# Kmatsuo57/cell-image-analysis

Hardware: AMD Instinct MI355X
Metric: cells/sec screened (CAE fwd + recon-MSE + SVM score), 64x64 (higher is better)
Workload: dtype f32 (results in the fp32 error class; the contractions run as split 16-bit products on the matrix pipe, fp32 accumulate: conv1..conv6 as 2 fp16 terms x 3 products with exact power-of-two scales from each cell's own data, the PCA GEMM as 3 bf16 terms x 6 products, conv7's 32 -> 16 channel contraction; 1 GPU; BASELINE.json configs[2]: screening inference, 1000000 synthetic 64x64 crops on one GPU, resident in HBM, CAE fwd + recon MSE/MAE + RobustScaler + PCA(100) + 2x OCSVM score on device; cells_per_gpu=1000000, global_cells=1000000, chunk_cells=65536, detector_train_cells=5000, weights=random init (Glorot, non-trivial BN), seed 42, parallelism=dp1

## Files before the change

### cell-image-analysis_amd/cellscreen/_lib.py

```python
from __future__ import annotations

import ctypes as C
import os
from typing import Optional

import numpy as np

CS_MAX_CONV = 16
CS_MEM_HOST, CS_MEM_DEVICE = 0, 1
_PKG = os.path.dirname(os.path.dirname(os.path.abspath(__file__)))
LIB_PATH = os.path.join(_PKG, "libcellscreen.so")


class CellScreenError(RuntimeError):
    def __init__(self, status: int, message: str):
        super().__init__(f"libcellscreen status {status}: {message}")
        self.status = status


class CSAugAffine(C.Structure):
    _fields_ = [("m", C.c_double * 4), ("off", C.c_double * 2), ("identity", C.c_int32), ("flip_h", C.c_int32),
                ("flip_v", C.c_int32), ("reserved", C.c_int32)]


# ... 24 lines not shown
                ("conservative", CSOcsvmParams), ("moderate", CSOcsvmParams)]


ALLGATHER_FN = C.CFUNCTYPE(C.c_int, C.c_void_p, C.c_int64)
ALLGATHER_STREAM_FN = C.CFUNCTYPE(C.c_int, C.c_void_p, C.c_int64, C.c_void_p)


class CSTrainCfg(C.Structure):
    _fields_ = [("beta1", C.c_float), ("beta2", C.c_float), ("adam_eps", C.c_float),
                ("bn_momentum", C.c_float), ("bn_eps", C.c_float)]


PRECISION_SPLIT16, PRECISION_FP32_EXACT = 0, 1
PRECISIONS = {"split16": PRECISION_SPLIT16, "fp32_exact": PRECISION_FP32_EXACT, "exact": PRECISION_FP32_EXACT,
              PRECISION_SPLIT16: PRECISION_SPLIT16, PRECISION_FP32_EXACT: PRECISION_FP32_EXACT}
DEBUG_NO_FUSE12, DEBUG_NO_FUSE45, DEBUG_NO_FUSE67, DEBUG_NO_SMALL_SPLIT = 1, 2, 4, 8


class CSModelOptions(C.Structure):
    _fields_ = [("struct_size", C.c_uint32), ("precision", C.c_int32), ("debug_flags", C.c_uint32), ("reserved", C.c_uint32 * 5)]


def model_options(precision="split16", debug_flags: int = 0) -> "CSModelOptions":
    if precision not in PRECISIONS:
        raise ValueError(f"precision must be 'split16' or 'fp32_exact', got {precision!r}")
    o = CSModelOptions()
    o.struct_size = C.sizeof(CSModelOptions)
    o.precision = PRECISIONS[precision]
    o.debug_flags = int(debug_flags)
    return o

# ... 335 lines not shown
```

### cell-image-analysis_amd/csrc/api.hip

```cpp
#include "api_internal.hpp"
#include "tensor_archive.hpp"

using namespace cs;

static thread_local std::string g_err;

namespace cs {
int fail(int code, const char* fmt, ...)
{
    char buf[1024];
    va_list ap;
    va_start(ap, fmt);
    vsnprintf(buf, sizeof buf, fmt, ap);
    va_end(ap);
    g_err = buf;
    return code;
}
const char* last_error_cstr() { return g_err.c_str(); }
}

static const char* kKernelNames[K_COUNT] = {"conv1_relu_bn_pool", "conv2_relu_bn_pool", "conv3_relu_bn_pool",
                                            "conv4_relu_bn",      "conv5_up_relu_bn",   "conv6_up_relu_bn",
                                            "conv7_up_sigmoid_err", "scaler_pca",       "ocsvm_decision",
                                            "finalize",           "synth_crops",        "conv6_conv7_fused_err",
                                            "conv1_conv2_fused"};

struct ConvSet {
    DevBuf winocs[3];
    DevBuf c12w1;
    DevBuf c3h2, c4h2, c5h2, c6h2;
    float c3h2_inv = 1.0f, c4h2_inv = 1.0f, c5h2_inv = 1.0f, c6h2_inv = 1.0f;
    DevBuf c12w1h2;
    float c12w1h2_inv = 1.0f;
    DevBuf c12h2;
    float c12h2_inv = 1.0f, p1a = 0.0f, p1b = 0.0f;
    DevBuf c12;
    DevBuf winoup[6];
    DevBuf wfrag[6];
    DevBuf ep[6];
    int n = 0;
};

struct GenSet {
    DevBuf w[CS_MAX_CONV], ep[CS_MAX_CONV], wf[CS_MAX_CONV], wx3[CS_MAX_CONV];
    bool folded[CS_MAX_CONV] = {false}, x3[CS_MAX_CONV] = {false};
    DevBuf wh2[CS_MAX_CONV];
// ... 15 lines not shown

constexpr int64_t kPackedResultCells = 65536;

struct cs_model {
    int device = 0;
    hipStream_t stream = nullptr;
    hipStream_t copy_stream = nullptr;
    hipEvent_t ev_in[2] = {nullptr, nullptr}, ev_used[2] = {nullptr, nullptr};
    Arch arch;
    ConvSet ae, enc;
    GenSet gae, genc;
    bool shared_encoder = true;
    int precision = CS_PRECISION_SPLIT16;
    unsigned debug_flags = 0;
    bool split16 = true;
    bool fuse12 = true, fuse45 = true, fuse67 = true, small_split = true;
    int errparts = 4;
    DevBuf w7eff, b7;
    bool has_det = false;
    int F = 0, fpad = 0, C = 0, cpad = 0;
    DevBuf center, scale, comps, comps_x3, mean_proj;
    struct Svm { DevBuf svT, svn, coef; int nsv = 0, nsv_pad = 0; double gamma = 0, rho = 0; } svm[2];
    int64_t chunk = 0;
    int64_t ws_cells = 0;
    DevBuf xin, xin2, act[CS_MAX_CONV], featE, pca, errpart, dec[2], o_mse, o_mae, o_sc[2], o_pr[2], recon;
    DevBuf det_ws;
    DevBuf o_pack;
    void* h_pack = nullptr;
    size_t h_pack_bytes = 0;
    bool prof = false;
    std::vector<ProfEvent> pending;
// ... 152 lines not shown
        }
        if (l == 4) {
            std::vector<float> weff(pack_generic_folded(cin, cout, nullptr, nullptr));
            pack_generic_folded(cin, cout, w->kernel[l], weff.data());
            std::vector<uint16_t> h2(pack_conv5_f16x2(nullptr, nullptr, nullptr));
            pack_conv5_f16x2(weff.data(), h2.data(), &set.c5h2_inv);
            rc = upload(set.c5h2, h2.data(), h2.size() * sizeof(uint16_t));
            if (rc) return rc;
        }
        if (l == 5) {
            std::vector<float> weff(pack_generic_folded(cin, cout, nullptr, nullptr));
            pack_generic_folded(cin, cout, w->kernel[l], weff.data());
            std::vector<uint16_t> h2(pack_conv6_f16x2(nullptr, nullptr, nullptr));
            pack_conv6_f16x2(weff.data(), h2.data(), &set.c6h2_inv);
            rc = upload(set.c6h2, h2.data(), h2.size() * sizeof(uint16_t));
            if (rc) return rc;
        }
        if (l == 0) {
            tmp.resize(pack_conv12_conv1_fragments(nullptr, nullptr, nullptr));
            pack_conv12_conv1_fragments(w->kernel[l], ep.data() + cout, tmp.data());
            rc = upload(set.c12w1, tmp.data(), tmp.size() * sizeof(float));
            if (rc) return rc;
            pack_conv12_p1_bound(w->kernel[l], ep.data(), &set.p1a, &set.p1b);
            std::vector<unsigned int> wh(pack_conv12_conv1_h2(nullptr, nullptr, nullptr, nullptr));
            pack_conv12_conv1_h2(w->kernel[l], ep.data() + cout, wh.data(), &set.c12w1h2_inv);
            rc = upload(set.c12w1h2, wh.data(), wh.size() * sizeof(unsigned int));
            if (rc) return rc;
        }
        if (l == 1) {
            tmp.resize(pack_conv12_fragments(nullptr, nullptr, nullptr));
// ... 260 lines not shown
        if (l == 1 || l == 2) {
            LAUNCH(K_CONV1 + l, nc,
                   launch_conv_wino_cs(l, in, set.winocs[l].as<float>(), set.ep[l].as<float>(), m->act[l].as<float>(), nc, m->stream));
            continue;
        }
        if (l == 3 && h2) {
            LAUNCH(K_CONV4, nc,
                   launch_conv4_h2(in, set.c4h2.as<uint16_t>(), set.c4h2_inv, set.ep[l].as<float>(), m->act[l].as<float>(), nc, m->stream));
            continue;
        }
        LAUNCH(K_CONV1 + l, nc,
               launch_conv_mfma(l, in, set.wfrag[l].as<float>(), set.ep[l].as<float>(), m->act[l].as<float>(), nc, m->stream, false));
    }
    if (fused && h2) {
        LAUNCH(K_CONV67_FUSED, nc,
               launch_conv67_h2(m->act[4].as<float>(), set.c6h2.as<uint16_t>(), set.c6h2_inv, set.ep[5].as<float>(), x, m->w7eff.as<float>(),
                                m->b7.as<float>(), m->errpart.as<float>(), nc, m->stream));
        m->errparts = conv67_fused_nparts();
    } else if (fused) {
        LAUNCH(K_CONV67_FUSED, nc,
               launch_conv67_fused(m->act[4].as<float>(), set.winoup[5].as<float>(), set.ep[5].as<float>(), x, m->w7eff.as<float>(),
                                   m->b7.as<float>(), m->errpart.as<float>(), nc, m->stream));
        m->errparts = conv67_fused_nparts();
    } else if (last >= 6) {
        LAUNCH(K_CONV7_ERR, nc,
               launch_conv7_err(m->act[5].as<float>(), x, m->w7eff.as<float>(), m->b7.as<float>(), m->errpart.as<float>(), recon, nc, m->stream));
        m->errparts = 4;
    }
    return CS_OK;
}

struct DrainGuard {
// ... 81 lines not shown
int cs_device_count(void)
{
    int n = 0;
    if (hipGetDeviceCount(&n) != hipSuccess) return 0;
    return n;
}

static int resolve_options(const cs_model_options* o, int* precision, unsigned* flags)
{
    *precision = CS_PRECISION_SPLIT16;
    *flags = 0;
    if (o) {
        if (o->struct_size < 12 || o->struct_size > 4096) return fail(CS_ERR_INVALID, "cs_model_options.struct_size = %u (set it to sizeof(cs_model_options))", o->struct_size);
        if (o->precision != CS_PRECISION_SPLIT16 && o->precision != CS_PRECISION_FP32_EXACT)
            return fail(CS_ERR_INVALID, "cs_model_options.precision = %d (CS_PRECISION_SPLIT16 or CS_PRECISION_FP32_EXACT)", o->precision);
        const unsigned known = CS_DEBUG_NO_FUSE12 | CS_DEBUG_NO_FUSE45 | CS_DEBUG_NO_FUSE67 | CS_DEBUG_NO_SMALL_SPLIT;
        if (o->debug_flags & ~known) return fail(CS_ERR_INVALID, "cs_model_options.debug_flags = 0x%x has unknown bits", o->debug_flags);
        if (o->struct_size >= sizeof(cs_model_options))
            for (unsigned r : o->reserved) if (r) return fail(CS_ERR_INVALID, "cs_model_options.reserved must be 0");
        *precision = o->precision;
        *flags = o->debug_flags;
    }
    if (const char* e = getenv("CS_DEBUG_PRECISION")) {
        if (!strcmp(e, "exact")) *precision = CS_PRECISION_FP32_EXACT;
        else if (!strcmp(e, "split16")) *precision = CS_PRECISION_SPLIT16;
        else return fail(CS_ERR_INVALID, "CS_DEBUG_PRECISION=%s (exact or split16)", e);
    }
    if (const char* e = getenv("CS_DEBUG_FLAGS")) *flags |= (unsigned)strtoul(e, nullptr, 0) & 0xfu;
    return CS_OK;
}

int cs_model_from_arrays(const cs_cae_weights* autoencoder, const cs_cae_weights* encoder,
                         const cs_detector_params* det, int device_id, const cs_model_options* options, cs_model** out)
{
    if (!out) return fail(CS_ERR_INVALID, "out is NULL");
    *out = nullptr;
    int precision;
    unsigned dflags;
    {
        int rco = resolve_options(options, &precision, &dflags);
        if (rco) return rco;
    }
    Arch arch;
// ... 2 lines not shown
    if (arch.ref && (rc = check_arch(autoencoder, kNConv, "autoencoder"))) return rc;
    if (encoder && (rc = check_encoder(encoder, arch))) return rc;
    if ((rc = require_gfx950(device_id))) return rc;

    cs_model* m = new (std::nothrow) cs_model();
    if (!m) return fail(CS_ERR_NOMEM, "host allocation failed");
    m->device = device_id;
    m->arch = arch;
    m->precision = precision;
    m->debug_flags = dflags;
    m->split16 = precision == CS_PRECISION_SPLIT16;
    m->fuse12 = !(dflags & CS_DEBUG_NO_FUSE12);
    m->fuse45 = !(dflags & CS_DEBUG_NO_FUSE45);
    m->fuse67 = !(dflags & CS_DEBUG_NO_FUSE67);
    m->small_split = !(dflags & CS_DEBUG_NO_SMALL_SPLIT);
#define FAIL_IF(x) do { int r__ = (x); if (r__) { delete m; return r__; } } while (0)
    {
        hipError_t e = hipStreamCreateWithFlags(&m->stream, hipStreamNonBlocking);
        if (e == hipSuccess) e = hipStreamCreateWithFlags(&m->copy_stream, hipStreamNonBlocking);
        for (int i = 0; i < 2 && e == hipSuccess; ++i) {
            e = hipEventCreateWithFlags(&m->ev_in[i], hipEventDisableTiming);
            if (e == hipSuccess) e = hipEventCreateWithFlags(&m->ev_used[i], hipEventDisableTiming);
        }
        if (e != hipSuccess) { delete m; return fail(CS_ERR_HIP, "stream/event creation: %s", hipGetErrorString(e)); }
    }
    if (arch.ref) {
        FAIL_IF(pack_set(m->ae, autoencoder, 6));
        float weff[16 * 32];
        conv7_effective_weights(autoencoder->kernel[6], weff);
        FAIL_IF(upload(m->w7eff, weff, sizeof weff));
// ... 549 lines not shown

int cs_profile_bf16_mfma_per_cell(cs_model* m, int k, double* mfma)
{
    if (!m || !mfma || k < 0 || k >= K_COUNT) return fail(CS_ERR_INVALID, "bad kernel id");
    double v = 0.0;
    if (!m->split16) { *mfma = 0.0; return CS_OK; }
    if (k == K_SCALER_PCA && m->has_det) {
        *mfma = (double)(m->cpad / 16) * (m->fpad / 32) * 6.0 / 16.0;
        return CS_OK;
    }
    if (m->arch.ref) {
        if (k == K_CONV4) v = 4 * 2 * 9 * 3;
        if (k == K_CONV3) v = 16.0 * 4 * 2 * 2 * 3;
        if (k == K_CONV12_FUSED) v = 66 * 8 * 2 + 36 * 4 * 4 * 3;
        if (k == K_CONV5) v = 4 * 4 * 4 * 4 * 3 + (m->fuse45 ? 4 * 2 * 9 * 3 : 0);
        if (k == K_CONV67_FUSED) v = 4.0 * 16 * 2 * 4 * 2 * 3;
    } else if (k <= K_CONV6) {
        const int l = k - K_CONV1;
        if (l < m->arch.n_conv && m->gae.x3[l]) {
            const int cout_pad = (m->arch.ch[l] + 15) / 16 * 16;
            const double taps = l > m->arch.n_enc ? 4.0 : 9.0;
            const bool last = l == m->arch.n_conv - 1;
            v = (double)m->arch.gh[l] * m->arch.gw[l] / 16.0 * (cout_pad / 16) * taps * (m->arch.cin(l) / 32.0) * ((m->gae.h2_inv[l] != 0.0f && !last) ? 3.0 : 6.0);
        }
    }
    *mfma = v;
    return CS_OK;
}

}
```

### cell-image-analysis_amd/csrc/common.hpp

```cpp
#pragma once
#include <hip/hip_runtime.h>
#include <stdint.h>
#include <stdio.h>

#include "../../include/cellscreen.h"

namespace cs {

typedef float f32x4 __attribute__((ext_vector_type(4)));

struct LayerGeom {
    int H, W, cin, cout;
    bool pool;
    bool ups;
    bool last;
};

enum KernelId {
    K_CONV1 = 0, K_CONV2, K_CONV3, K_CONV4, K_CONV5, K_CONV6, K_CONV7_ERR,
    K_SCALER_PCA, K_SVM, K_FINALIZE, K_SYNTH, K_CONV67_FUSED, K_CONV12_FUSED, K_COUNT
};

hipError_t launch_conv_mfma(int layer, const float* in, const float* wfrag, const float* ep,
                            float* out, int64_t n_cells, hipStream_t stream, bool folded = false);
// ... 14 lines not shown
size_t pack_conv12_conv1_fragments(const float* hwio, const float* bn_scale, float* dst);
hipError_t launch_conv4_h2(const float* in, const uint16_t* wfrag, float inv_sw, const float* ep, float* out, int64_t n_cells, hipStream_t stream);
size_t pack_conv4_f16x2(const float* hwio, uint16_t* dst, float* inv_sw);
hipError_t launch_conv5_h2(const float* in, const uint16_t* wfrag, float inv_sw, const float* ep, float* out, int64_t n_cells, hipStream_t stream);
hipError_t launch_conv45_h2(const float* in, const uint16_t* w4, float inv_sw4, const float* ep4, const uint16_t* w5, float inv_sw5,
                            const float* ep5, float* out, int64_t n_cells, hipStream_t stream);
size_t pack_conv5_f16x2(const float* weff, uint16_t* dst, float* inv_sw);
hipError_t launch_conv_wino_up(int layer, const float* in, const float* ufrag, const float* ep, float* out, int64_t n_cells,
                               hipStream_t stream);
size_t pack_wino_up_fragments(int layer, const float* hwio, float* dst);
size_t pack_conv_fragments(int cin, int cout, const float* hwio, float* dst);

hipError_t launch_conv67_fused(const float* a5, const float* ufrag, const float* ep, const float* x, const float* weff_dev,
                               const float* b7_dev, float* errpart, int64_t n_cells, hipStream_t stream);
int conv67_fused_nparts();
hipError_t launch_conv67_h2(const float* a5, const uint16_t* wplanes, float inv_sw, const float* ep, const float* x, const float* weff_dev,
                            const float* b7_dev, float* errpart, int64_t n_cells, hipStream_t stream);
size_t pack_conv6_f16x2(const float* weff, uint16_t* dst, float* inv_sw);

hipError_t launch_conv7_err(const float* a6, const float* x, const float* weff_dev, const float* b7_dev,
                            float* errpart, float* recon, int64_t n_cells, hipStream_t stream);
hipError_t launch_conv7_err_train(const float* a6, const float* x, const float* weff_dev, const float* b7_dev, float* errpart,
                                  float* recon, float* dz, float* dzsum_part, int64_t n_cells, hipStream_t stream);
void conv7_effective_weights(const float* w7_hwio, float* weff);

constexpr int TRAIN_MAX_PARTS = 256;
constexpr int BN_MAX_PARTS = 1024;
struct ReduceDesc { long dst; long len; const float* src; int nparts; long stride; };
hipError_t launch_conv_train_fwd(int layer, const float* in, const float* wfrag, const float* bias,
                                 float* relu_out, int64_t n_cells, hipStream_t stream, float* stats_part = nullptr,
                                 int* stats_parts = nullptr);
hipError_t launch_conv_dgrad(int layer, const float* dz, const float* wfrag_t, float* dx, int64_t n_cells,
                             hipStream_t stream);
// ... 84 lines not shown
```

### cell-image-analysis_amd/csrc/conv_wino_up.hip

```cpp
#include "kernel_setup.hpp"
#include "split16.hpp"

#include <type_traits>

#include <cmath>
#include <cstdlib>
#include <cstring>

namespace cs {

namespace {

template <int HS_, int WS_, int CIN_, int COUT_>
struct WUCfg {
    static constexpr int HS = HS_, WS = WS_, CIN = CIN_, COUT = COUT_;
    static constexpr int HO = 2 * HS, WO = 2 * WS;
    static constexpr int TW = WS / 2;
    static constexpr int SR = 2 * (16 / TW);
    static constexpr int R = SR + 2, WP = WS + 2;
    static constexpr int PS = CIN + 4;
    static constexpr int STRIP = R * WP * PS * 4;
    static constexpr int LDS = 2 * STRIP;
    static constexpr int NGRP = HS / SR;
    static constexpr int NQ = CIN / 16, KS = CIN / 4;
// ... 393 lines not shown

struct F67H {
    static constexpr int PLB = 2 * 64;
    static constexpr int PXB = 2 * PLB + 32;
    static constexpr int ROWB = 18 * PXB;
    static constexpr int STRIP = 6 * ROWB;
    static constexpr int TW = F67T::TW;
    static constexpr int T_BYTES = F67T::T_BYTES;
    static constexpr int PA = 40;
    static constexpr int A6_BYTES = 8 * 32 * PA * 4;
    static constexpr int WP = 40;
    static constexpr int W_BYTES = 16 * WP * 4;
    static constexpr int OFF_MAX = STRIP + A6_BYTES + T_BYTES + W_BYTES;
    static constexpr int LDS = OFF_MAX + 16;
    static_assert(LDS <= 160 * 1024 && STRIP % 16 == 0, "LDS budget");
};

__device__ __forceinline__ void h2_store(char* strip, int j, int rsub, int loffb, const f32x4& v, float S)
{
    const int r = rsub + WUL6::RPP * j;
    f16x4 hi, lo;
    f16x2_split4(v, S, hi, lo);
    char* d = strip + r * F67H::ROWB + loffb;
    *(f16x4*)d = hi;
    *(f16x4*)(d + F67H::PLB) = lo;
}

__device__ __forceinline__ f32x4 h2_prep(int y0, int j, int rsub, f32x4 v, unsigned int& mx)
{
    const int sy = y0 - 1 + rsub + WUL6::RPP * j;
    if (sy < 0 || sy >= WUL6::HS) v = f32x4{0.0f, 0.0f, 0.0f, 0.0f};
    f16x2_absmax4(v, mx);
    return v;
}

template <bool DIAG>
__global__ __launch_bounds__(WUL6::THREADS, 2) void conv67_h2_kernel(
    const float* __restrict__ in , const f16x8* __restrict__ wfrag, const float* __restrict__ ep ,
    const float* __restrict__ x , const float* __restrict__ weff ,
    const float* __restrict__ b7p, float* __restrict__ errpart , long n_cells, float inv_sw,
    unsigned long long* __restrict__ diag)
{
    using C = WUL6;
    static_assert(C::NLD == 3 && C::RPP == 2 && C::R == 6 && C::EPR == 256, "row-wise staging constants");
    unsigned long long dg[5] = {0, 0, 0, 0, 0}, dt = 0;
    extern __shared__ __attribute__((aligned(16))) char smem[];
    float* a6s = (float*)(smem + F67H::STRIP);
    float* tb = (float*)(smem + F67H::STRIP + F67H::A6_BYTES);
    float* wl = (float*)(smem + F67H::STRIP + F67H::A6_BYTES + F67H::T_BYTES);
    unsigned int* mxw = (unsigned int*)(smem + F67H::OFF_MAX);
    const int tid = threadIdx.x, lane = tid & 63;
    const int wave = __builtin_amdgcn_readfirstlane(tid >> 6);
    const int ph = wave >> 1, wsl = wave & 1;
    const int pa = ph >> 1, pb = ph & 1;
    const int li = lane & 15, kq = lane >> 4;

    f16x8 B[4][2][2];
#pragma unroll
    for (int t = 0; t < 4; ++t)
#pragma unroll
        for (int k = 0; k < 2; ++k)
#pragma unroll
            for (int p = 0; p < 2; ++p) B[t][k][p] = wfrag[(((wave * 4 + t) * 2 + k) * 2 + p) * 64 + lane];
    const int co = wsl * 16 + li;
    const int cosw = co ^ ((kq & 1) << 4);
    const float bias = ep[co], bns = ep[C::COUT + co], bnt = ep[2 * C::COUT + co];
    const float b7 = b7p[0];

    const long first = blockIdx.x;
    if (first >= n_cells) return;
    const int se = tid & (C::EPR - 1), rsub = tid / C::EPR;
    const int spx = se / C::C4, sc4 = se & (C::C4 - 1);
    const int goff = spx * C::CIN + sc4 * 4;
    const int loffb = (spx + 1) * F67H::PXB + sc4 * 8;
    auto cell_ptr = [&](long cell) { return in + (size_t)cell * C::HS * C::WS * C::CIN; };
    for (int i = tid; i < F67H::LDS / 16; i += C::THREADS) ((f32x4*)smem)[i] = f32x4{0.0f, 0.0f, 0.0f, 0.0f};
    __syncthreads();
    wl[(tid >> 5) * F67H::WP + (tid & 31)] = weff[tid];
    float unscale;
    {
        f32x4 stg[C::NLD];
        unsigned int mx = 0;
#pragma unroll
        for (int j = 0; j < C::NLD; ++j) stg[j] = h2_prep(0, j, rsub, wu_load<C>(cell_ptr(first), 0, j, rsub, goff), mx);
        mx = f16x2_rowmax(mx);
        if (li == 0) atomicMax(&mxw[0], mx);
        __syncthreads();
        float S, invS;
        f16x2_scale(mxw[0], S, invS);
        unscale = invS * inv_sw;
#pragma unroll
        for (int j = 0; j < C::NLD; ++j) h2_store(smem, j, rsub, loffb, stg[j], S);
    }
    __syncthreads();
    if (tid == 0) mxw[0] = 0;
    const char* abase = smem + (pa * 18 + li + pb) * F67H::PXB + kq * 16;

    int strip_no = 0;
    for (long cell = first; cell < n_cells; cell += gridDim.x) {
        const float* xc = x + (size_t)cell * 64 * 64;
        float s2 = 0.0f, s1 = 0.0f;
#pragma unroll 1
        for (int grp = 0; grp < C::NGRP; ++grp) {
            const long ncell = grp < C::NGRP - 1 ? cell : cell + gridDim.x;
            const int ngrp = grp < C::NGRP - 1 ? grp + 1 : 0;
            const bool has_next = ncell < n_cells;
            ++strip_no;
            unsigned int* const mword = mxw + (strip_no & 1);

            if constexpr (DIAG) dt = cycle_stamp();
            f32x4 stg[C::NLD];
            if (has_next) {
#pragma unroll
                for (int j = 0; j < C::NLD; ++j) stg[j] = wu_load<C>(cell_ptr(ncell), ngrp * C::SR, j, rsub, goff);
            }
            float xv[2];
#pragma unroll
            for (int h = 0; h < 2; ++h) {
                const int k = wave + 8 * h, o = 2 * (8 * grp + (k >> 1)) - 1 + (k & 1);
                xv[h] = xc[(o < 0 ? 0 : o) * 64 + lane];
            }
            float xtail = 0.0f;
            if (grp == C::NGRP - 1 && wave == 0) xtail = xc[63 * 64 + lane];

            if constexpr (DIAG) { const unsigned long long t = cycle_stamp(); dg[0] += t - dt; dt = t; }
            f32x4 ah[4], al[4];
#pragma unroll
            for (int t = 0; t < 4; ++t) ah[t] = al[t] = f32x4{0.0f, 0.0f, 0.0f, 0.0f};
            auto rd = [&](int f, f16x8 (&a)[2]) {
                const int sr = f >> 2, rx = (f >> 1) & 1, k = f & 1;
                const char* p = abase + sr * F67H::ROWB + rx * F67H::PXB + k * 64;
                a[0] = *(const f16x8*)p;
                a[1] = *(const f16x8*)(p + F67H::PLB);
            };
            auto mac3 = [&](const f16x8 (&a)[2], const f16x8 (&b)[2], f32x4& dh, f32x4& dl) {
                dl = __builtin_amdgcn_mfma_f32_16x16x32_f16(a[0], b[1], dl, 0, 0, 0);
                dh = __builtin_amdgcn_mfma_f32_16x16x32_f16(a[0], b[0], dh, 0, 0, 0);
                dl = __builtin_amdgcn_mfma_f32_16x16x32_f16(a[1], b[0], dl, 0, 0, 0);
            };
            {
// ... 12 lines not shown
                    if (sr > 0 && sr < 4) __builtin_amdgcn_sched_group_barrier(0x008, 6, 0);
                    else __builtin_amdgcn_sched_group_barrier(0x008, 3, 0);
                }
            }
            if constexpr (DIAG) {
                asm volatile("" ::"v"(ah[0][0]), "v"(al[3][3]));
                const unsigned long long t = cycle_stamp(); dg[1] += t - dt; dt = t;
            }
#pragma unroll
            for (int t = 0; t < 4; ++t)
#pragma unroll
                for (int r = 0; r < 4; ++r) {
                    const float v = fmaxf(fmaf(ah[t][r] + al[t][r], unscale, bias), 0.0f);
                    a6s[((2 * t + pa) * 32 + 2 * (4 * kq + r) + pb) * F67H::PA + cosw] = fmaf(v, bns, bnt);
                }
            if (has_next) {
                unsigned int mx = 0;
#pragma unroll
                for (int j = 0; j < C::NLD; ++j) stg[j] = h2_prep(ngrp * C::SR, j, rsub, stg[j], mx);
                mx = f16x2_rowmax(mx);
                if (li == 0) atomicMax(mword, mx);
            }
            __syncthreads();
            if constexpr (DIAG) { const unsigned long long t = cycle_stamp(); dg[2] += t - dt; dt = t; }
            {
                const int wrow = 4 * ((li >> 3) | (((li >> 2) & 1) << 1)) + (li & 3);
                float wc[8];
                *(f32x4*)&wc[0] = *(const f32x4*)(wl + wrow * F67H::WP + 4 * kq);
                *(f32x4*)&wc[4] = *(const f32x4*)(wl + wrow * F67H::WP + 4 * kq + 16);
                const int pix = 4 * (li & 3) + (li >> 2), sw = ((li >> 1) & 1) << 4;
                const float* ap = a6s + (wave * 32 + pix) * F67H::PA + 4 * kq;
                const f32x4 a00 = *(const f32x4*)(ap + sw), a01 = *(const f32x4*)(ap + (sw ^ 16));
                const f32x4 a10 = *(const f32x4*)(ap + 16 * F67H::PA + sw), a11 = *(const f32x4*)(ap + 16 * F67H::PA + (sw ^ 16));
                f32x4 t0 = f32x4{0.0f, 0.0f, 0.0f, 0.0f}, t1 = t0;
#pragma unroll
                for (int s = 0; s < 4; ++s) {
                    t0 = __builtin_amdgcn_mfma_f32_16x16x4f32(wc[s], a00[s], t0, 0, 0, 0);
                    t1 = __builtin_amdgcn_mfma_f32_16x16x4f32(wc[s], a10[s], t1, 0, 0, 0);
                }
#pragma unroll
                for (int s = 0; s < 4; ++s) {
                    t0 = __builtin_amdgcn_mfma_f32_16x16x4f32(wc[4 + s], a01[s], t0, 0, 0, 0);
                    t1 = __builtin_amdgcn_mfma_f32_16x16x4f32(wc[4 + s], a11[s], t1, 0, 0, 0);
                }
                const int rblk = kq == 0 ? 0 : (kq == 1 ? 3 : (kq == 2 ? 1 : 2));
                float* tw = tb + ((((8 * grp + wave) & (F67::TSLOTS - 1)) * 16) + 4 * rblk) * F67H::TW + pix + 1 - (kq >> 1);
#pragma unroll
                for (int r = 0; r < 4; ++r) { tw[r * F67H::TW] = t0[r]; tw[r * F67H::TW + 16] = t1[r]; }
            }
            if (has_next) {
                float S, invS;
                f16x2_scale(*mword, S, invS);
                unscale = invS * inv_sw;
#pragma unroll
                for (int j = 0; j < C::NLD; ++j) h2_store(smem, j, rsub, loffb, stg[j], S);
            }
            __syncthreads();
            if (tid == 0) *mword = 0;
            if constexpr (DIAG) { const unsigned long long t = cycle_stamp(); dg[3] += t - dt; dt = t; }
            const int px = lane & 1, xh = lane >> 1;
#pragma unroll
            for (int h = 0; h < 2; ++h) {
                const int k = wave + 8 * h;
                const int y = 8 * grp + (k >> 1), e = k & 1;
                if (2 * y - 1 + e < 0) continue;
                const int nb = (e ? px : 3 - px) * 4;
                const float* ra = tb + ((((y - 1) & (F67::TSLOTS - 1)) * 16) + nb) * F67H::TW + xh;
                const float* rb = tb + (((y & (F67::TSLOTS - 1)) * 16) + nb) * F67H::TW + xh;
// ... 8 lines not shown
            }
            if (grp == C::NGRP - 1 && wave == 0) {
                const int nb = (3 - px) * 4;
                const float* ra = tb + (((31 & (F67::TSLOTS - 1)) * 16) + nb) * F67H::TW + xh;
                const float v = (ra[0] + ra[F67H::TW + 1]) + b7;
                const float rr = f67_sigmoid(v);
                const float d = xtail - rr;
                s2 = fmaf(d, d, s2);
                s1 += fabsf(d);
            }
            if constexpr (DIAG) {
                asm volatile("" ::"v"(s2), "v"(s1));
                const unsigned long long t = cycle_stamp(); dg[4] += t - dt; dt = t;
            }
        }
#pragma unroll
        for (int off = 32; off > 0; off >>= 1) {
            s2 += __shfl_down(s2, off, 64);
            s1 += __shfl_down(s1, off, 64);
        }
        if (lane == 0) {
            errpart[((size_t)cell * F67::NPARTS + wave) * 2 + 0] = s2;
            errpart[((size_t)cell * F67::NPARTS + wave) * 2 + 1] = s1;
        }
    }
    if constexpr (DIAG) {
        if (lane == 0) {
#pragma unroll
            for (int k = 0; k < 5; ++k) diag[((size_t)blockIdx.x * 8 + wave) * 5 + k] = dg[k];
        }
    }
}

template <class C>
// ... 80 lines not shown
    if (inv_sw) *inv_sw = 1.0f / S;
    for (int w = 0; w < 8; ++w)
        for (int t = 0; t < 4; ++t)
            for (int k = 0; k < 2; ++k)
                for (int l = 0; l < 64; ++l)
                    for (int j = 0; j < 8; ++j) {
                        const int ph = w >> 1, half = w & 1, li = l & 15, kq = l >> 4;
                        const float v = weff[((size_t)(ph * 4 + t) * 64 + 32 * k + 8 * kq + j) * 32 + 16 * half + li];
                        uint16_t pl[2];
                        f16x2_split(v, S, pl[0], pl[1]);
                        for (int p = 0; p < 2; ++p) dst[((((((size_t)w * 4 + t) * 2 + k) * 2 + p) * 64) + l) * 8 + j] = pl[p];
                    }
    return n;
}

hipError_t launch_conv67_h2(const float* a5, const uint16_t* wplanes, float inv_sw, const float* ep, const float* x, const float* weff_dev,
                            const float* b7_dev, float* errpart, int64_t n_cells, hipStream_t stream)
{
    static const bool diag = getenv("CS_WINO_DIAG") != nullptr;
    KernelSetup ks;
    const hipError_t e = !diag ? kernel_setup<conv67_h2_kernel<false>>(WUL6::THREADS, F67H::LDS, ks)
                               : kernel_setup<conv67_h2_kernel<true>>(WUL6::THREADS, F67H::LDS, ks, &g_wu_stamps[0]);
    if (e != hipSuccess) return e;
    if (n_cells <= 0) return hipSuccess;
    const unsigned grid = (unsigned)(n_cells < ks.cus ? n_cells : ks.cus);
    if (diag)
        hipLaunchKernelGGL(conv67_h2_kernel<true>, dim3(grid), dim3(WUL6::THREADS), F67H::LDS, stream, a5, (const f16x8*)wplanes, ep, x,
                           weff_dev, b7_dev, errpart, (long)n_cells, inv_sw, g_wu_stamps[0].begin(ks, grid));
    else
        hipLaunchKernelGGL(conv67_h2_kernel<false>, dim3(grid), dim3(WUL6::THREADS), F67H::LDS, stream, a5, (const f16x8*)wplanes, ep, x,
                           weff_dev, b7_dev, errpart, (long)n_cells, inv_sw, (unsigned long long*)nullptr);
    return hipGetLastError();
}

size_t pack_wino_up_fragments(int layer, const float* hwio, float* dst)
{
    return layer == 5 ? pack_frags<WUL6>(hwio, dst) : pack_frags<WUL5>(hwio, dst);
}

hipError_t launch_conv_wino_up(int layer, const float* in, const float* ufrag, const float* ep, float* out, int64_t n_cells,
                               hipStream_t stream)
{
    if (layer == 5) return launch<WUL6>(layer, in, ufrag, ep, out, n_cells, stream);
    if (layer == 4) return launch<WUL5>(layer, in, ufrag, ep, out, n_cells, stream);
    return hipErrorInvalidValue;
}

}

extern "C" int cs_debug_wino_up_diag(int layer, double out5[5])
{
    if (layer < 3 || layer > 5) return -1;
    return cs::stamp_table_average(cs::g_wu_stamps[layer - 3], 5, out5);
}
```

### include/cellscreen.h

```cpp
#ifndef CELLSCREEN_H
#define CELLSCREEN_H

#include <stdint.h>

#ifdef __cplusplus
extern "C" {
#endif

#define CS_ABI_VERSION 2
#define CS_MAX_CONV 16

typedef enum cs_status {
    CS_OK = 0,
    CS_ERR_INVALID = -1,
    CS_ERR_IO = -2,
    CS_ERR_FORMAT = -3,
    CS_ERR_NO_DEVICE = -4,
    CS_ERR_HIP = -5,
    CS_ERR_UNSUPPORTED = -6,
    CS_ERR_NOMEM = -7,
    CS_ERR_NO_DETECTOR = -8
} cs_status;

typedef enum cs_mem_kind { CS_MEM_HOST = 0, CS_MEM_DEVICE = 1 } cs_mem_kind;
// ... 26 lines not shown
    int32_t n_components;
    const float *scaler_center;
    const double *scaler_scale;
    const float *pca_components;
    const float *pca_mean_proj;
    cs_ocsvm_params conservative;
    cs_ocsvm_params moderate;
} cs_detector_params;

typedef enum cs_precision { CS_PRECISION_SPLIT16 = 0, CS_PRECISION_FP32_EXACT = 1 } cs_precision;

#define CS_DEBUG_NO_FUSE12      0x1u
#define CS_DEBUG_NO_FUSE45      0x2u
#define CS_DEBUG_NO_FUSE67      0x4u
#define CS_DEBUG_NO_SMALL_SPLIT 0x8u

typedef struct cs_model_options {
    uint32_t struct_size;
    int32_t precision;
    uint32_t debug_flags;
    uint32_t reserved[5];
} cs_model_options;

typedef struct cs_model_info {
    int32_t height, width;
    int32_t n_conv, n_enc;
    int32_t feature_dim;
    int32_t n_components;
    int32_t n_sv_conservative, n_sv_moderate;
    int32_t shared_encoder;
// ... 456 lines not shown
```

Before: 5.563 million cells/s.

## Compute fused conv6 upsample as nine direct taps with cross-wave halo exchange

Adds a new default path for the fused conv6+conv7 kernel. It packs the conv6 weights per tap (9 taps) instead of the folded 4-phase sub-pixel form. Each wave computes tap products on its input row, combines horizontal neighbours with DPP lane shifts, and swaps vertical halo rows with other waves through a new LDS area. The aim is to cut the MFMA count per cell relative to the folded-phase formulation. The change also adds a swizzled LDS channel layout, epilogue params staged in LDS and a ds_swizzle reduction, at the cost of more LDS, an extra barrier and more complex scale handling across groups.

New measurement: 5.506 million cells/s. -1.0%, worse.

```diff
diff --git a/cell-image-analysis_amd/cellscreen/_lib.py b/cell-image-analysis_amd/cellscreen/_lib.py
--- a/cell-image-analysis_amd/cellscreen/_lib.py
+++ b/cell-image-analysis_amd/cellscreen/_lib.py
@@ -62,7 +62,7 @@
 PRECISION_SPLIT16, PRECISION_FP32_EXACT = 0, 1
 PRECISIONS = {"split16": PRECISION_SPLIT16, "fp32_exact": PRECISION_FP32_EXACT, "exact": PRECISION_FP32_EXACT,
               PRECISION_SPLIT16: PRECISION_SPLIT16, PRECISION_FP32_EXACT: PRECISION_FP32_EXACT}
-DEBUG_NO_FUSE12, DEBUG_NO_FUSE45, DEBUG_NO_FUSE67, DEBUG_NO_SMALL_SPLIT = 1, 2, 4, 8
+DEBUG_NO_FUSE12, DEBUG_NO_FUSE45, DEBUG_NO_FUSE67, DEBUG_NO_SMALL_SPLIT, DEBUG_NO_TAPS67 = 1, 2, 4, 8, 0x20
 
 
 class CSModelOptions(C.Structure):
diff --git a/cell-image-analysis_amd/csrc/api.hip b/cell-image-analysis_amd/csrc/api.hip
--- a/cell-image-analysis_amd/csrc/api.hip
+++ b/cell-image-analysis_amd/csrc/api.hip
@@ -30,6 +30,8 @@
     DevBuf c12w1;
     DevBuf c3h2, c4h2, c5h2, c6h2;
     float c3h2_inv = 1.0f, c4h2_inv = 1.0f, c5h2_inv = 1.0f, c6h2_inv = 1.0f;
+    DevBuf c6t;
+    float c6t_inv = 1.0f;
     DevBuf c12w1h2;
     float c12w1h2_inv = 1.0f;
     DevBuf c12h2;
@@ -75,7 +77,7 @@
     int precision = CS_PRECISION_SPLIT16;
     unsigned debug_flags = 0;
     bool split16 = true;
-    bool fuse12 = true, fuse45 = true, fuse67 = true, small_split = true;
+    bool fuse12 = true, fuse45 = true, fuse67 = true, small_split = true, taps67 = true;
     int errparts = 4;
     DevBuf w7eff, b7;
     bool has_det = false;
@@ -258,6 +260,10 @@
             std::vector<uint16_t> h2(pack_conv6_f16x2(nullptr, nullptr, nullptr));
             pack_conv6_f16x2(weff.data(), h2.data(), &set.c6h2_inv);
             rc = upload(set.c6h2, h2.data(), h2.size() * sizeof(uint16_t));
+            if (rc) return rc;
+            std::vector<uint16_t> t9(pack_conv6_taps_f16x2(nullptr, nullptr, nullptr));
+            pack_conv6_taps_f16x2(w->kernel[l], t9.data(), &set.c6t_inv);
+            rc = upload(set.c6t, t9.data(), t9.size() * sizeof(uint16_t));
             if (rc) return rc;
         }
         if (l == 0) {
@@ -548,8 +554,8 @@
     }
     if (fused && h2) {
         LAUNCH(K_CONV67_FUSED, nc,
-               launch_conv67_h2(m->act[4].as<float>(), set.c6h2.as<uint16_t>(), set.c6h2_inv, set.ep[5].as<float>(), x, m->w7eff.as<float>(),
-                                m->b7.as<float>(), m->errpart.as<float>(), nc, m->stream));
+               launch_conv67_h2(m->act[4].as<float>(), (m->taps67 ? set.c6t : set.c6h2).as<uint16_t>(), m->taps67 ? set.c6t_inv : set.c6h2_inv,
+                                m->taps67, set.ep[5].as<float>(), x, m->w7eff.as<float>(), m->b7.as<float>(), m->errpart.as<float>(), nc, m->stream));
         m->errparts = conv67_fused_nparts();
     } else if (fused) {
         LAUNCH(K_CONV67_FUSED, nc,
@@ -661,7 +667,7 @@
         if (o->struct_size < 12 || o->struct_size > 4096) return fail(CS_ERR_INVALID, "cs_model_options.struct_size = %u (set it to sizeof(cs_model_options))", o->struct_size);
         if (o->precision != CS_PRECISION_SPLIT16 && o->precision != CS_PRECISION_FP32_EXACT)
             return fail(CS_ERR_INVALID, "cs_model_options.precision = %d (CS_PRECISION_SPLIT16 or CS_PRECISION_FP32_EXACT)", o->precision);
-        const unsigned known = CS_DEBUG_NO_FUSE12 | CS_DEBUG_NO_FUSE45 | CS_DEBUG_NO_FUSE67 | CS_DEBUG_NO_SMALL_SPLIT;
+        const unsigned known = CS_DEBUG_NO_FUSE12 | CS_DEBUG_NO_FUSE45 | CS_DEBUG_NO_FUSE67 | CS_DEBUG_NO_SMALL_SPLIT | CS_DEBUG_NO_TAPS67;
         if (o->debug_flags & ~known) return fail(CS_ERR_INVALID, "cs_model_options.debug_flags = 0x%x has unknown bits", o->debug_flags);
         if (o->struct_size >= sizeof(cs_model_options))
             for (unsigned r : o->reserved) if (r) return fail(CS_ERR_INVALID, "cs_model_options.reserved must be 0");
@@ -673,7 +679,7 @@
         else if (!strcmp(e, "split16")) *precision = CS_PRECISION_SPLIT16;
         else return fail(CS_ERR_INVALID, "CS_DEBUG_PRECISION=%s (exact or split16)", e);
     }
-    if (const char* e = getenv("CS_DEBUG_FLAGS")) *flags |= (unsigned)strtoul(e, nullptr, 0) & 0xfu;
+    if (const char* e = getenv("CS_DEBUG_FLAGS")) *flags |= (unsigned)strtoul(e, nullptr, 0) & 0x2fu;
     return CS_OK;
 }
 
@@ -706,6 +712,7 @@
     m->fuse45 = !(dflags & CS_DEBUG_NO_FUSE45);
     m->fuse67 = !(dflags & CS_DEBUG_NO_FUSE67);
     m->small_split = !(dflags & CS_DEBUG_NO_SMALL_SPLIT);
+    m->taps67 = !(dflags & CS_DEBUG_NO_TAPS67);
 #define FAIL_IF(x) do { int r__ = (x); if (r__) { delete m; return r__; } } while (0)
     {
         hipError_t e = hipStreamCreateWithFlags(&m->stream, hipStreamNonBlocking);
@@ -1285,7 +1292,7 @@
         if (k == K_CONV3) v = 16.0 * 4 * 2 * 2 * 3;
         if (k == K_CONV12_FUSED) v = 66 * 8 * 2 + 36 * 4 * 4 * 3;
         if (k == K_CONV5) v = 4 * 4 * 4 * 4 * 3 + (m->fuse45 ? 4 * 2 * 9 * 3 : 0);
-        if (k == K_CONV67_FUSED) v = 4.0 * 16 * 2 * 4 * 2 * 3;
+        if (k == K_CONV67_FUSED) v = conv67_h2_mfma_per_cell(m->taps67);
     } else if (k <= K_CONV6) {
         const int l = k - K_CONV1;
         if (l < m->arch.n_conv && m->gae.x3[l]) {
diff --git a/cell-image-analysis_amd/csrc/common.hpp b/cell-image-analysis_amd/csrc/common.hpp
--- a/cell-image-analysis_amd/csrc/common.hpp
+++ b/cell-image-analysis_amd/csrc/common.hpp
@@ -52,9 +52,11 @@
 hipError_t launch_conv67_fused(const float* a5, const float* ufrag, const float* ep, const float* x, const float* weff_dev,
                                const float* b7_dev, float* errpart, int64_t n_cells, hipStream_t stream);
 int conv67_fused_nparts();
-hipError_t launch_conv67_h2(const float* a5, const uint16_t* wplanes, float inv_sw, const float* ep, const float* x, const float* weff_dev,
-                            const float* b7_dev, float* errpart, int64_t n_cells, hipStream_t stream);
+hipError_t launch_conv67_h2(const float* a5, const uint16_t* wplanes, float inv_sw, bool taps, const float* ep, const float* x,
+                            const float* weff_dev, const float* b7_dev, float* errpart, int64_t n_cells, hipStream_t stream);
 size_t pack_conv6_f16x2(const float* weff, uint16_t* dst, float* inv_sw);
+size_t pack_conv6_taps_f16x2(const float* hwio, uint16_t* dst, float* inv_sw);
+int conv67_h2_mfma_per_cell(bool taps);
 
 hipError_t launch_conv7_err(const float* a6, const float* x, const float* weff_dev, const float* b7_dev,
                             float* errpart, float* recon, int64_t n_cells, hipStream_t stream);
diff --git a/cell-image-analysis_amd/csrc/conv_wino_up.hip b/cell-image-analysis_amd/csrc/conv_wino_up.hip
--- a/cell-image-analysis_amd/csrc/conv_wino_up.hip
+++ b/cell-image-analysis_amd/csrc/conv_wino_up.hip
@@ -431,7 +431,37 @@
     static constexpr int OFF_MAX = STRIP + A6_BYTES + T_BYTES + W_BYTES;
     static constexpr int LDS = OFF_MAX + 16;
     static_assert(LDS <= 160 * 1024 && STRIP % 16 == 0, "LDS budget");
+    __device__ static __forceinline__ int chan(int col, int c0) { return c0 ^ (((col >> 3) & 1) << 4); }
 };
+
+struct F67N {
+    static constexpr int PA = 32;
+    static constexpr int A6_BYTES = 8 * 32 * PA * 4;
+    static constexpr int XCH_SLOT = 64 * 16;
+    static constexpr int XCH_BYTES = 34 * XCH_SLOT;
+    static constexpr int OFF_XCH = F67H::STRIP + A6_BYTES + F67H::T_BYTES + F67H::W_BYTES;
+    static constexpr int OFF_EP = OFF_XCH + XCH_BYTES;
+    static constexpr int OFF_MAX = OFF_EP + 3 * 32 * 4;
+    static constexpr int LDS = OFF_MAX + 16;
+    static constexpr int MFMA_PER_CELL = 4 * (8 * 54 + 2 * 18);
+    static_assert(LDS <= 160 * 1024, "LDS budget");
+    __device__ static __forceinline__ int chan(int col, int c0)
+    {
+        return c0 ^ ((((col >> 2) & 1) << 2) | (((col >> 1) & 1) << 3) | (((col >> 3) & 1) << 4));
+    }
+};
+
+template <bool SHR>
+__device__ __forceinline__ float row_neighbour(float v)
+{
+    return __builtin_bit_cast(float, __builtin_amdgcn_update_dpp(0, __builtin_bit_cast(int, v), SHR ? 0x111 : 0x101, 0xf, 0xf, true));
+}
+
+template <int M>
+__device__ __forceinline__ float lane_xor(float v)
+{
+    return __builtin_bit_cast(float, __builtin_amdgcn_ds_swizzle(__builtin_bit_cast(int, v), (M << 10) | 0x1f));
+}
 
 __device__ __forceinline__ void h2_store(char* strip, int j, int rsub, int loffb, const f32x4& v, float S)
 {
@@ -451,7 +481,7 @@
     return v;
 }
 
-template <bool DIAG>
+template <bool DIAG, bool TAPS>
 __global__ __launch_bounds__(WUL6::THREADS, 2) void conv67_h2_kernel(
     const float* __restrict__ in , const f16x8* __restrict__ wfrag, const float* __restrict__ ep ,
     const float* __restrict__ x , const float* __restrict__ weff ,
@@ -459,28 +489,30 @@
     unsigned long long* __restrict__ diag)
 {
     using C = WUL6;
+    using L = std::conditional_t<TAPS, F67N, F67H>;
     static_assert(C::NLD == 3 && C::RPP == 2 && C::R == 6 && C::EPR == 256, "row-wise staging constants");
     unsigned long long dg[5] = {0, 0, 0, 0, 0}, dt = 0;
     extern __shared__ __attribute__((aligned(16))) char smem[];
     float* a6s = (float*)(smem + F67H::STRIP);
-    float* tb = (float*)(smem + F67H::STRIP + F67H::A6_BYTES);
-    float* wl = (float*)(smem + F67H::STRIP + F67H::A6_BYTES + F67H::T_BYTES);
-    unsigned int* mxw = (unsigned int*)(smem + F67H::OFF_MAX);
+    float* tb = (float*)(smem + F67H::STRIP + L::A6_BYTES);
+    float* wl = (float*)(smem + F67H::STRIP + L::A6_BYTES + F67H::T_BYTES);
+    unsigned int* mxw = (unsigned int*)(smem + L::OFF_MAX);
     const int tid = threadIdx.x, lane = tid & 63;
     const int wave = __builtin_amdgcn_readfirstlane(tid >> 6);
     const int ph = wave >> 1, wsl = wave & 1;
     const int pa = ph >> 1, pb = ph & 1;
     const int li = lane & 15, kq = lane >> 4;
 
-    f16x8 B[4][2][2];
-#pragma unroll
-    for (int t = 0; t < 4; ++t)
+    constexpr int NT = TAPS ? 9 : 4;
+    f16x8 B[NT][2][2];
+#pragma unroll
+    for (int t = 0; t < NT; ++t)
 #pragma unroll
         for (int k = 0; k < 2; ++k)
 #pragma unroll
-            for (int p = 0; p < 2; ++p) B[t][k][p] = wfrag[(((wave * 4 + t) * 2 + k) * 2 + p) * 64 + lane];
+            for (int p = 0; p < 2; ++p) B[t][k][p] = wfrag[((((TAPS ? wsl : wave) * NT + t) * 2 + k) * 2 + p) * 64 + lane];
     const int co = wsl * 16 + li;
-    const int cosw = co ^ ((kq & 1) << 4);
+    const int cosw = F67H::chan(8 * kq, co);
     const float bias = ep[co], bns = ep[C::COUT + co], bnt = ep[2 * C::COUT + co];
     const float b7 = b7p[0];
 
@@ -491,9 +523,12 @@
     const int goff = spx * C::CIN + sc4 * 4;
     const int loffb = (spx + 1) * F67H::PXB + sc4 * 8;
     auto cell_ptr = [&](long cell) { return in + (size_t)cell * C::HS * C::WS * C::CIN; };
-    for (int i = tid; i < F67H::LDS / 16; i += C::THREADS) ((f32x4*)smem)[i] = f32x4{0.0f, 0.0f, 0.0f, 0.0f};
+    for (int i = tid; i < L::LDS / 16; i += C::THREADS) ((f32x4*)smem)[i] = f32x4{0.0f, 0.0f, 0.0f, 0.0f};
     __syncthreads();
     wl[(tid >> 5) * F67H::WP + (tid & 31)] = weff[tid];
+    if constexpr (TAPS) {
+        if (tid < 3 * C::COUT) ((float*)(smem + F67N::OFF_EP))[tid] = ep[tid];
+    }
     float unscale;
     {
         f32x4 stg[C::NLD];
@@ -505,13 +540,15 @@
         __syncthreads();
         float S, invS;
         f16x2_scale(mxw[0], S, invS);
-        unscale = invS * inv_sw;
+        unscale = TAPS ? __builtin_bit_cast(float, __builtin_amdgcn_readfirstlane(__builtin_bit_cast(int, invS * inv_sw))) : invS * inv_sw;
 #pragma unroll
         for (int j = 0; j < C::NLD; ++j) h2_store(smem, j, rsub, loffb, stg[j], S);
     }
     __syncthreads();
     if (tid == 0) mxw[0] = 0;
-    const char* abase = smem + (pa * 18 + li + pb) * F67H::PXB + kq * 16;
+    const char* abase = TAPS ? smem + ((ph + 1) * 18 + li + 1) * F67H::PXB + kq * 16 : smem + (pa * 18 + li + pb) * F67H::PXB + kq * 16;
+    f32x4* const xch = (f32x4*)(smem + F67N::OFF_XCH) + lane;
+    float* const a6w = a6s + (2 * ph * 32 + 2 * li) * F67N::PA + F67N::chan(2 * li, 16 * wsl + 4 * kq);
 
     int strip_no = 0;
     for (long cell = first; cell < n_cells; cell += gridDim.x) {
@@ -531,16 +568,112 @@
 #pragma unroll
                 for (int j = 0; j < C::NLD; ++j) stg[j] = wu_load<C>(cell_ptr(ncell), ngrp * C::SR, j, rsub, goff);
             }
-            float xv[2];
-#pragma unroll
-            for (int h = 0; h < 2; ++h) {
-                const int k = wave + 8 * h, o = 2 * (8 * grp + (k >> 1)) - 1 + (k & 1);
-                xv[h] = xc[(o < 0 ? 0 : o) * 64 + lane];
-            }
-            float xtail = 0.0f;
-            if (grp == C::NGRP - 1 && wave == 0) xtail = xc[63 * 64 + lane];
+            float xv[2], xtail = 0.0f;
+            auto load_x = [&]() {
+#pragma unroll
+                for (int h = 0; h < 2; ++h) {
+                    const int k = wave + 8 * h, o = 2 * (8 * grp + (k >> 1)) - 1 + (k & 1);
+                    xv[h] = xc[(unsigned)((o < 0 ? 0 : o) * 64 + lane)];
+                }
+                if constexpr (TAPS) {
+                    if (wave == 0) xtail = xc[(unsigned)((16 * grp + 15) * 64 + lane)];
+                } else if (grp == C::NGRP - 1 && wave == 0) xtail = xc[63 * 64 + lane];
+            };
+            if constexpr (!TAPS) load_x();
 
             if constexpr (DIAG) { const unsigned long long t = cycle_stamp(); dg[0] += t - dt; dt = t; }
+            if constexpr (TAPS) {
+            const int t = ph;
+            f16x8 xa[2][2];
+#pragma unroll
+            for (int k = 0; k < 2; ++k)
+#pragma unroll
+                for (int p = 0; p < 2; ++p) xa[k][p] = *(const f16x8*)(abase + k * 64 + p * F67H::PLB);
+            f32x4 z[9];
+#pragma unroll
+            for (int j = 0; j < 9; ++j) z[j] = f32x4{0.0f, 0.0f, 0.0f, 0.0f};
+#pragma unroll
+            for (int s = 0; s < 3; ++s)
+#pragma unroll
+                for (int k = 0; k < 2; ++k)
+#pragma unroll
+                    for (int j = 0; j < 9; ++j)
+                        z[j] = __builtin_amdgcn_mfma_f32_16x16x32_f16(B[j][k][s == 0], xa[k][s == 1], z[j], 0, 0, 0);
+            f32x4 c[3][2];
+#pragma unroll
+            for (int i = 0; i < 3; ++i)
+#pragma unroll
+                for (int r = 0; r < 4; ++r) {
+                    c[i][0][r] = row_neighbour<true>(z[3 * i][r]) + (z[3 * i + 1][r] + z[3 * i + 2][r]);
+                    c[i][1][r] = (z[3 * i][r] + z[3 * i + 1][r]) + row_neighbour<false>(z[3 * i + 2][r]);
+                }
+            {
+                const int s0 = t < 3 ? (t * 2 + wsl) * 2 : 12 + ((grp & 1) * 2 + wsl) * 2;
+                const float cs = t < 3 ? 1.0f : unscale;
+                xch[64 * s0] = c[0][0] * cs;
+                xch[64 * (s0 + 1)] = c[0][1] * cs;
+                if (t > 0) {
+                    xch[64 * (20 + ((t - 1) * 2 + wsl) * 2)] = c[2][0];
+                    xch[64 * (20 + ((t - 1) * 2 + wsl) * 2 + 1)] = c[2][1];
+                }
+            }
+            f32x4 up[2], dn[2];
+            if (t == 3) {
+#pragma unroll
+                for (int k = 0; k < 2; ++k)
+#pragma unroll
+                    for (int p = 0; p < 2; ++p) xa[k][p] = *(const f16x8*)(abase + F67H::ROWB + k * 64 + p * F67H::PLB);
+                f32x4 zh[3];
+#pragma unroll
+                for (int j = 0; j < 3; ++j) zh[j] = f32x4{0.0f, 0.0f, 0.0f, 0.0f};
+#pragma unroll
+                for (int s = 0; s < 3; ++s)
+#pragma unroll
+                    for (int k = 0; k < 2; ++k)
+#pragma unroll
+                        for (int j = 0; j < 3; ++j)
+                            zh[j] = __builtin_amdgcn_mfma_f32_16x16x32_f16(B[6 + j][k][s == 0], xa[k][s == 1], zh[j], 0, 0, 0);
+#pragma unroll
+                for (int r = 0; r < 4; ++r) {
+                    dn[0][r] = row_neighbour<true>(zh[0][r]) + (zh[1][r] + zh[2][r]);
+                    dn[1][r] = (zh[0][r] + zh[1][r]) + row_neighbour<false>(zh[2][r]);
+                }
+            }
+            if constexpr (DIAG) {
+                asm volatile("" ::"v"(c[1][0][0]), "v"(c[1][1][3]));
+                const unsigned long long ts = cycle_stamp(); dg[1] += ts - dt; dt = ts;
+            }
+            __syncthreads();
+            {
+                const int su = t > 0 ? ((t - 1) * 2 + wsl) * 2 : (grp > 0 ? 12 + (((grp - 1) & 1) * 2 + wsl) * 2 : 32);
+                up[0] = xch[64 * su];
+                up[1] = xch[64 * (su + 1)];
+                if (t == 0 && grp > 0) {
+                    const float rs = __builtin_bit_cast(float, 0x7f000000u - __builtin_bit_cast(unsigned int, unscale));
+                    up[0] *= rs;
+                    up[1] *= rs;
+                }
+            }
+            if (t < 3) {
+                dn[0] = xch[64 * (20 + (t * 2 + wsl) * 2)];
+                dn[1] = xch[64 * (20 + (t * 2 + wsl) * 2 + 1)];
+            }
+            const f32x4* const ep4 = (const f32x4*)(smem + F67N::OFF_EP) + 4 * wsl + kq;
+            const f32x4 bias4 = ep4[0], bns4 = ep4[8], bnt4 = ep4[16];
+#pragma unroll
+            for (int a = 0; a < 2; ++a)
+#pragma unroll
+                for (int b = 0; b < 2; ++b) {
+                    f32x4 o;
+#pragma unroll
+                    for (int r = 0; r < 4; ++r) {
+                        const float s = a == 0 ? up[b][r] + (c[1][b][r] + c[2][b][r]) : (c[0][b][r] + c[1][b][r]) + dn[b][r];
+                        o[r] = fmaf(fmaxf(fmaf(s, unscale, bias4[r]), 0.0f), bns4[r], bnt4[r]);
+                    }
+                    *(f32x4*)(a6w + (a * 32 + b) * F67N::PA) = o;
+                }
+            load_x();
+            } else {
             f32x4 ah[4], al[4];
 #pragma unroll
             for (int t = 0; t < 4; ++t) ah[t] = al[t] = f32x4{0.0f, 0.0f, 0.0f, 0.0f};
@@ -583,6 +716,7 @@
                     const float v = fmaxf(fmaf(ah[t][r] + al[t][r], unscale, bias), 0.0f);
                     a6s[((2 * t + pa) * 32 + 2 * (4 * kq + r) + pb) * F67H::PA + cosw] = fmaf(v, bns, bnt);
                 }
+            }
             if (has_next) {
                 unsigned int mx = 0;
 #pragma unroll
@@ -597,10 +731,10 @@
                 float wc[8];
                 *(f32x4*)&wc[0] = *(const f32x4*)(wl + wrow * F67H::WP + 4 * kq);
                 *(f32x4*)&wc[4] = *(const f32x4*)(wl + wrow * F67H::WP + 4 * kq + 16);
-                const int pix = 4 * (li & 3) + (li >> 2), sw = ((li >> 1) & 1) << 4;
-                const float* ap = a6s + (wave * 32 + pix) * F67H::PA + 4 * kq;
+                const int pix = 4 * (li & 3) + (li >> 2), sw = L::chan(pix, 4 * kq);
+                const float* ap = a6s + (wave * 32 + pix) * L::PA;
                 const f32x4 a00 = *(const f32x4*)(ap + sw), a01 = *(const f32x4*)(ap + (sw ^ 16));
-                const f32x4 a10 = *(const f32x4*)(ap + 16 * F67H::PA + sw), a11 = *(const f32x4*)(ap + 16 * F67H::PA + (sw ^ 16));
+                const f32x4 a10 = *(const f32x4*)(ap + 16 * L::PA + sw), a11 = *(const f32x4*)(ap + 16 * L::PA + (sw ^ 16));
                 f32x4 t0 = f32x4{0.0f, 0.0f, 0.0f, 0.0f}, t1 = t0;
 #pragma unroll
                 for (int s = 0; s < 4; ++s) {
@@ -620,7 +754,7 @@
             if (has_next) {
                 float S, invS;
                 f16x2_scale(*mword, S, invS);
-                unscale = invS * inv_sw;
+                unscale = TAPS ? __builtin_bit_cast(float, __builtin_amdgcn_readfirstlane(__builtin_bit_cast(int, invS * inv_sw))) : invS * inv_sw;
 #pragma unroll
                 for (int j = 0; j < C::NLD; ++j) h2_store(smem, j, rsub, loffb, stg[j], S);
             }
@@ -659,10 +793,20 @@
                 const unsigned long long t = cycle_stamp(); dg[4] += t - dt; dt = t;
             }
         }
-#pragma unroll
-        for (int off = 32; off > 0; off >>= 1) {
-            s2 += __shfl_down(s2, off, 64);
-            s1 += __shfl_down(s1, off, 64);
+        if constexpr (TAPS) {
+            s2 += __shfl_down(s2, 32, 64);
+            s1 += __shfl_down(s1, 32, 64);
+            s2 += lane_xor<16>(s2); s1 += lane_xor<16>(s1);
+            s2 += lane_xor<8>(s2); s1 += lane_xor<8>(s1);
+            s2 += lane_xor<4>(s2); s1 += lane_xor<4>(s1);
+            s2 += lane_xor<2>(s2); s1 += lane_xor<2>(s1);
+            s2 += lane_xor<1>(s2); s1 += lane_xor<1>(s1);
+        } else {
+#pragma unroll
+            for (int off = 32; off > 0; off >>= 1) {
+                s2 += __shfl_down(s2, off, 64);
+                s1 += __shfl_down(s1, off, 64);
+            }
         }
         if (lane == 0) {
             errpart[((size_t)cell * F67::NPARTS + wave) * 2 + 0] = s2;
@@ -773,23 +917,54 @@
     return n;
 }
 
-hipError_t launch_conv67_h2(const float* a5, const uint16_t* wplanes, float inv_sw, const float* ep, const float* x, const float* weff_dev,
-                            const float* b7_dev, float* errpart, int64_t n_cells, hipStream_t stream)
+size_t pack_conv6_taps_f16x2(const float* hwio, uint16_t* dst, float* inv_sw)
+{
+    const size_t n = (size_t)2 * 9 * 2 * 2 * 64 * 8;
+    if (!dst) return n;
+    const float S = f16x2_weight_scale(hwio, (size_t)9 * 64 * 32);
+    if (inv_sw) *inv_sw = 1.0f / S;
+    for (int half = 0; half < 2; ++half)
+        for (int t = 0; t < 9; ++t)
+            for (int k = 0; k < 2; ++k)
+                for (int l = 0; l < 64; ++l)
+                    for (int j = 0; j < 8; ++j) {
+                        const int li = l & 15, kq = l >> 4;
+                        const float v = hwio[((size_t)t * 64 + 32 * k + 8 * kq + j) * 32 + 16 * half + li];
+                        uint16_t pl[2];
+                        f16x2_split(v, S, pl[0], pl[1]);
+                        for (int p = 0; p < 2; ++p) dst[((((((size_t)half * 9 + t) * 2 + k) * 2 + p) * 64) + l) * 8 + j] = pl[p];
+                    }
+    return n;
+}
+
+int conv67_h2_mfma_per_cell(bool taps) { return taps ? F67N::MFMA_PER_CELL : 4 * 16 * 2 * 4 * 2 * 3; }
+
+template <bool TAPS>
+static hipError_t launch67_h2(const float* a5, const uint16_t* wplanes, float inv_sw, const float* ep, const float* x, const float* weff_dev,
+                              const float* b7_dev, float* errpart, int64_t n_cells, hipStream_t stream)
 {
     static const bool diag = getenv("CS_WINO_DIAG") != nullptr;
+    constexpr int LDSB = TAPS ? F67N::LDS : F67H::LDS;
     KernelSetup ks;
-    const hipError_t e = !diag ? kernel_setup<conv67_h2_kernel<false>>(WUL6::THREADS, F67H::LDS, ks)
-                               : kernel_setup<conv67_h2_kernel<true>>(WUL6::THREADS, F67H::LDS, ks, &g_wu_stamps[0]);
+    const hipError_t e = !diag ? kernel_setup<conv67_h2_kernel<false, TAPS>>(WUL6::THREADS, LDSB, ks)
+                               : kernel_setup<conv67_h2_kernel<true, TAPS>>(WUL6::THREADS, LDSB, ks, &g_wu_stamps[0]);
     if (e != hipSuccess) return e;
     if (n_cells <= 0) return hipSuccess;
     const unsigned grid = (unsigned)(n_cells < ks.cus ? n_cells : ks.cus);
     if (diag)
-        hipLaunchKernelGGL(conv67_h2_kernel<true>, dim3(grid), dim3(WUL6::THREADS), F67H::LDS, stream, a5, (const f16x8*)wplanes, ep, x,
+        hipLaunchKernelGGL((conv67_h2_kernel<true, TAPS>), dim3(grid), dim3(WUL6::THREADS), LDSB, stream, a5, (const f16x8*)wplanes, ep, x,
                            weff_dev, b7_dev, errpart, (long)n_cells, inv_sw, g_wu_stamps[0].begin(ks, grid));
     else
-        hipLaunchKernelGGL(conv67_h2_kernel<false>, dim3(grid), dim3(WUL6::THREADS), F67H::LDS, stream, a5, (const f16x8*)wplanes, ep, x,
+        hipLaunchKernelGGL((conv67_h2_kernel<false, TAPS>), dim3(grid), dim3(WUL6::THREADS), LDSB, stream, a5, (const f16x8*)wplanes, ep, x,
                            weff_dev, b7_dev, errpart, (long)n_cells, inv_sw, (unsigned long long*)nullptr);
     return hipGetLastError();
+}
+
+hipError_t launch_conv67_h2(const float* a5, const uint16_t* wplanes, float inv_sw, bool taps, const float* ep, const float* x,
+                            const float* weff_dev, const float* b7_dev, float* errpart, int64_t n_cells, hipStream_t stream)
+{
+    return taps ? launch67_h2<true>(a5, wplanes, inv_sw, ep, x, weff_dev, b7_dev, errpart, n_cells, stream)
+                : launch67_h2<false>(a5, wplanes, inv_sw, ep, x, weff_dev, b7_dev, errpart, n_cells, stream);
 }
 
 size_t pack_wino_up_fragments(int layer, const float* hwio, float* dst)
@@ -812,3 +987,11 @@
     if (layer < 3 || layer > 5) return -1;
     return cs::stamp_table_average(cs::g_wu_stamps[layer - 3], 5, out5);
 }
+
+extern "C" int cs_debug_conv67_workgroups(int taps)
+{
+    cs::KernelSetup ks;
+    const hipError_t e = taps ? cs::kernel_setup<cs::conv67_h2_kernel<false, true>>(cs::WUL6::THREADS, cs::F67N::LDS, ks)
+                              : cs::kernel_setup<cs::conv67_h2_kernel<false, false>>(cs::WUL6::THREADS, cs::F67H::LDS, ks);
+    return e == hipSuccess ? ks.cus : -1;
+}
diff --git a/include/cellscreen.h b/include/cellscreen.h
--- a/include/cellscreen.h
+++ b/include/cellscreen.h
@@ -64,6 +64,7 @@
 #define CS_DEBUG_NO_FUSE45      0x2u
 #define CS_DEBUG_NO_FUSE67      0x4u
 #define CS_DEBUG_NO_SMALL_SPLIT 0x8u
+#define CS_DEBUG_NO_TAPS67      0x20u
 
 typedef struct cs_model_options {
     uint32_t struct_size;
```
